# taindp98/Endoscopy-Image-Classification

Measured on AMD Instinct MI355X. Metric: unlabeled images/sec/node (FixMatch ViT-S, 224², μ=7), higher is better.
Workload: dtype bf16; 1 GPU; F1: FixMatch ViT-S/16 step, global B=64 labeled + mu*B=448 unlabeled weak/strong pairs (64 + 448 per GPU, strong scaling), 224^2, C=23, tau=0.95, lambda_u=1, Adam 1e-3, EMA 0.999; global_batch=960, seq_len=197, parallelism=dp1, hipgraph=False

## Files before the change

endoscopy-image-classification_amd/csrc/gemm.hip:

```cpp
#include <algorithm>
#include <cstdlib>

#include <hip/hip_ext.h>

#include "common.h"

namespace es_gemm {

constexpr int BM = 128, BN = 128, BK = 64;

enum Epi {
  EPI_BF16 = 0,
  EPI_GELU = 1,
  EPI_F32_RESID = 2,
  EPI_DGELU = 3,
  EPI_F32 = 4,
  EPI_PATCH = 5,
  EPI_GELU_ACT = 6,
  EPI_GELU_D = 7,
  EPI_MULAUX = 8,
};

struct NTArgs {
  const bf16* A; const bf16* B; const float* bias;
  void* C; void* C2; const void* aux;
  int M, N, K, lda, ldb, ldc, ldaux, np;
};

__device__ __forceinline__ int swz128(int r, int c) { return c ^ ((r >> 1) & 7); }
__device__ __forceinline__ int swz64(int r, int c) { return c ^ ((4 - ((r >> 2) & 3)) & 3); }

template <int EPI>
struct EpiCtx {
  __amdgpu_buffer_rsrc_t c, c2, aux;
// ... 1293 lines not shown
    if (d == (int)gridDim.x - 1) {
      for (int x = 0; x < 8; ++x)
        for (int c = 0; c < ncg; ++c) __hip_atomic_store(ctr + x * 8 + c, 0, __ATOMIC_RELAXED, __HIP_MEMORY_SCOPE_AGENT);
      __hip_atomic_store(ctr + SLOT_INTS - 1, 0, __ATOMIC_RELAXED, __HIP_MEMORY_SCOPE_AGENT);
    }
  }
}

namespace rlg {
constexpr int R = 32, KD = 384, D = 384;
constexpr int ROWA = KD * 2, TA = R * ROWA;
constexpr int ROWX = D * 4, TX = R * ROWX;
constexpr int STAGE = TA + TX, NST = 2;
constexpr int PA = TA / 1024 / 8, PX = TX / 1024 / 8;
constexpr int QN = 4;
constexpr int LDS = NST * STAGE + QN * 4 + 16 + D * 4 * 3;
constexpr int SLOTS = 64, SLOT_INTS = 4;
}
__device__ int g_rl_ctr[rlg::SLOTS * rlg::SLOT_INTS];

__device__ __forceinline__ float sq2_rounded(float a, float b) {
#pragma clang fp contract(off)
  return a * a + b * b;
}
__device__ __forceinline__ float sq2_fused(float a, float b) {
#pragma clang fp contract(off)
  return __builtin_fmaf(a, a, b * b);
}
__device__ __forceinline__ float mul_rounded(float a, float b) {
#pragma clang fp contract(off)
  return a * b;
}

struct RLArgs {
  const float* gamma; const float* beta;
  bf16* h; float* mean; float* rstd;
  int ldh; float eps;
};

__global__ __launch_bounds__(512, 1) void gemm_resid_ln_kernel(NTArgs p, RLArgs l, int slot) {
  using namespace rlg;
  extern __shared__ __attribute__((aligned(16))) char smem[];
  int* const qring = (int*)(smem + NST * STAGE);
  float* const bias_lds = (float*)(qring + QN + 4);
  float* const gam_lds = bias_lds + D;
  float* const bet_lds = gam_lds + D;
  const int tid = threadIdx.x, lane = tid & 63;
  const int w = __builtin_amdgcn_readfirstlane(tid >> 6);
  const int g = lane >> 4, r = lane & 15;
  int* const ctr = g_rl_ctr + slot * SLOT_INTS;
  const int nt = (p.M + R - 1) / R;
  if (tid == 0) {
    qring[0] = __hip_atomic_fetch_add(ctr, 1, __ATOMIC_RELAXED, __HIP_MEMORY_SCOPE_AGENT);
    qring[1] = __hip_atomic_fetch_add(ctr, 1, __ATOMIC_RELAXED, __HIP_MEMORY_SCOPE_AGENT);
  }
  bf16x8 wf[3][12];
  const int nw = w * 48;
#pragma unroll
  for (int j = 0; j < 3; ++j)
#pragma unroll
    for (int kk = 0; kk < 12; ++kk)
      wf[j][kk] = *(const bf16x8*)(p.B + (size_t)(nw + 16 * j + r) * p.ldb + 32 * kk + 8 * g);
  if (tid < D / 4) {
    *(f32x4*)(bias_lds + 4 * tid) = p.bias ? *(const f32x4*)(p.bias + 4 * tid) : f32x4{0.f, 0.f, 0.f, 0.f};
    *(f32x4*)(gam_lds + 4 * tid) = *(const f32x4*)(l.gamma + 4 * tid);
    *(f32x4*)(bet_lds + 4 * tid) = *(const f32x4*)(l.beta + 4 * tid);
// ... 72 lines not shown
        seq += 1;
        after_claim = seq;
      }
      char* S = smem + st * STAGE;
      unsigned xb4[4];
#pragma unroll
      for (int k = 0; k < 4; ++k)
        xb4[k] = (unsigned)(uintptr_t)(const __attribute__((address_space(3))) void*)(S + xbase[k]);
      f32x4 acc[2][3];
      ws_mfma_half<0>(acc, wf, xb4);
      ws_mfma_half<1>(acc, wf, xb4);
      char* X = S + TA;
#pragma unroll
      for (int a = 0; a < 2; ++a)
#pragma unroll
        for (int j = 0; j < 3; ++j) {
          const int row = 16 * a + r, c = w * 12 + 4 * j + g;
          f32x4* q = (f32x4*)(X + row * ROWX + ((c ^ r) << 4));
          const f32x4 v = acc[a][j] + *(const f32x4*)(bias_lds + nw + 16 * j + 4 * g);
          *q = v + *q;
        }
      asm volatile("s_waitcnt lgkmcnt(0)" ::: "memory");
      __builtin_amdgcn_s_barrier();
      const int m0 = cur * R;
#pragma unroll
      for (int q = 0; q < 4; ++q) {
        const int row = w * 4 + q;
        float2 v[3];
#pragma unroll
        for (int j = 0; j < 3; ++j) {
          const int cc = (j * 64 + lane) >> 1;
          v[j] = *(const float2*)(X + row * ROWX + ((cc ^ (row & 15)) << 4) + (lane & 1) * 8);
        }
        float s = 0.f;
#pragma unroll
        for (int j = 0; j < 3; ++j) s += v[j].x + v[j].y;
        const float mean = warp_sum(s) * (1.0f / D);
        float a[3], b[3];
#pragma unroll
        for (int j = 0; j < 3; ++j) {
          a[j] = v[j].x - mean;
          b[j] = v[j].y - mean;
        }
        const bool even = (q & 1) == 0;
        const float t0 = even ? sq2_fused(a[0], b[0]) : sq2_rounded(a[0], b[0]);
        const float t1 = sq2_rounded(a[1], b[1]);
        const float t2 = even ? sq2_fused(a[2], b[2]) : sq2_rounded(a[2], b[2]);
        const float ss = (t0 + t1) + t2;
        const float rstd = 1.0f / sqrtf(__builtin_fmaf(warp_sum(ss), 1.0f / D, l.eps));
        const int m = m0 + row;
        const bool ok = m < p.M;
#pragma unroll
        for (int j = 0; j < 3; ++j) {
          const int c = (j * 64 + lane) * 2;
          const float2 gm = *(const float2*)(gam_lds + c), bt = *(const float2*)(bet_lds + c);
          typedef __bf16 bf16x2 __attribute__((ext_vector_type(2)));
          bf16x2 o = {(bf16)__builtin_fmaf(mul_rounded(a[j], rstd), gm.x, bt.x),
                      (bf16)__builtin_fmaf(mul_rounded(b[j], rstd), gm.y, bt.y)};
          __builtin_amdgcn_raw_buffer_store_b64(__builtin_bit_cast(u32x2, v[j]), rx,
                                                ok ? (unsigned)(m * p.ldc + c) * 4u : ES_OOB, 0, 0);
          __builtin_amdgcn_raw_buffer_store_b32(__builtin_bit_cast(unsigned, o), rh,
                                                ok ? (unsigned)(m * l.ldh + c) * 2u : ES_OOB, 0, 0);
        }
        const bool one = ok && lane == 0;
        __builtin_amdgcn_raw_buffer_store_b32(__builtin_bit_cast(unsigned, mean), rm, one ? (unsigned)m * 4u : ES_OOB,
                                              0, 0);
        __builtin_amdgcn_raw_buffer_store_b32(__builtin_bit_cast(unsigned, rstd), rs, one ? (unsigned)m * 4u : ES_OOB,
                                              0, 0);
      }
      seq += 4 * 8;
      if (claimer) {
        wait_vmcnt_any(seq - after_claim);
        asm volatile("" : "+v"(claimed));
        const int c2 = __builtin_amdgcn_readfirstlane(claimed);
        if (lane == 0) qring[(it + 2) & (QN - 1)] = c2;
      }
      st ^= 1;
    }
  }
  asm volatile("s_waitcnt vmcnt(0)" ::: "memory");
  if (tid == 0) {
    const int d = __hip_atomic_fetch_add(ctr + SLOT_INTS - 1, 1, __ATOMIC_RELAXED, __HIP_MEMORY_SCOPE_AGENT);
    if (d == (int)gridDim.x - 1) {
      __hip_atomic_store(ctr, 0, __ATOMIC_RELAXED, __HIP_MEMORY_SCOPE_AGENT);
      __hip_atomic_store(ctr + SLOT_INTS - 1, 0, __ATOMIC_RELAXED, __HIP_MEMORY_SCOPE_AGENT);
    }
  }
}

#define NT_LAUNCH(E, BKT_, NST_, TBM_, ...)                                             \
  {                                                                                        \
    const size_t lds = std::max((size_t)NST_ * (TBM_ + BN) * BKT_ * 2, (size_t)4 * EPI_WAVE_BYTES); \
    allow_lds(gemm_nt_kernel<E, BKT_, NST_, TBM_, ##__VA_ARGS__>, lds);                   \
    hipLaunchKernelGGL(HIP_KERNEL_NAME(gemm_nt_kernel<E, BKT_, NST_, TBM_, ##__VA_ARGS__>), dim3(grid), dim3(256), lds, stream, a); \
    return ES_OK;                                                                          \
  }
#define NT_EPIS(BKT_, NST_, TBM_, ...)                                            \
  switch (epi) {                                                                  \
    case EPI_BF16: NT_LAUNCH(EPI_BF16, BKT_, NST_, TBM_, ##__VA_ARGS__)           \
    case EPI_GELU: NT_LAUNCH(EPI_GELU, BKT_, NST_, TBM_, ##__VA_ARGS__)           \
    case EPI_F32_RESID: NT_LAUNCH(EPI_F32_RESID, BKT_, NST_, TBM_, ##__VA_ARGS__) \
    case EPI_DGELU: NT_LAUNCH(EPI_DGELU, BKT_, NST_, TBM_, ##__VA_ARGS__)         \
    case EPI_F32: NT_LAUNCH(EPI_F32, BKT_, NST_, TBM_, ##__VA_ARGS__)             \
    case EPI_PATCH: NT_LAUNCH(EPI_PATCH, BKT_, NST_, TBM_, ##__VA_ARGS__)         \
    case EPI_GELU_ACT: NT_LAUNCH(EPI_GELU_ACT, BKT_, NST_, TBM_, ##__VA_ARGS__)   \
    case EPI_GELU_D: NT_LAUNCH(EPI_GELU_D, BKT_, NST_, TBM_, ##__VA_ARGS__)       \
    case EPI_MULAUX: NT_LAUNCH(EPI_MULAUX, BKT_, NST_, TBM_, ##__VA_ARGS__)       \
    default: return ES_BAD_ARG;                                                   \
  }
int launch_nt(int cfg, int epi, int grid, hipStream_t stream, const NTArgs& a) {
  if (cfg == 11 && epi == EPI_F32_RESID) NT_LAUNCH(EPI_F32_RESID, 64, 2, 64, 0)
// ... 69 lines not shown
    (void)hipGetDevice(&dev);
    if (hipDeviceGetAttribute(&cus, hipDeviceAttributeMultiprocessorCount, dev) != hipSuccess || cus <= 0) cus = 256;
  }
  const int ncg = a.N / wsg::NG;
  const int nrt = (a.M + wsg::R - 1) / wsg::R, nch = (nrt + wsg::CH - 1) / wsg::CH;
  const int per = std::max(1, std::min(cus / ncg, nch));
  const int grid = per * ncg;
  const int slot = ws_slot(stream);
  static const int probe = getenv("ENDOSSL_WS_PROBE") ? atoi(getenv("ENDOSSL_WS_PROBE")) : 0;
  if (probe == 5 && epi == EPI_BF16) WS_LAUNCH(EPI_BF16, 0, 5)
  if (probe == 7 && epi == EPI_BF16) WS_LAUNCH(EPI_BF16, 0, 7)
  switch (epi) {
    case EPI_BF16: WS_LAUNCH(EPI_BF16, 0)
    case EPI_GELU: WS_LAUNCH(EPI_GELU, 0)
    case EPI_GELU_ACT: WS_LAUNCH(EPI_GELU_ACT, 0)
    case EPI_GELU_D: WS_LAUNCH(EPI_GELU_D, 0)
    case EPI_F32: WS_LAUNCH(EPI_F32, 0)
    default: return ES_BAD_ARG;
  }
}
#undef WS_LAUNCH

int launch_resid_ln(hipStream_t stream, const NTArgs& a, const RLArgs& l) {
  static int cus = 0;
  if (!cus) {
    int dev = 0;
    (void)hipGetDevice(&dev);
    if (hipDeviceGetAttribute(&cus, hipDeviceAttributeMultiprocessorCount, dev) != hipSuccess || cus <= 0) cus = 256;
  }
  const int nt = (a.M + rlg::R - 1) / rlg::R;
  const int grid = std::max(1, std::min(cus, nt));
  allow_lds(gemm_resid_ln_kernel, (size_t)rlg::LDS);
  hipLaunchKernelGGL(gemm_resid_ln_kernel, dim3(grid), dim3(512), rlg::LDS, stream, a, l, ws_slot(stream));
  return hipGetLastError() == hipSuccess ? ES_OK : ES_HIP_ERROR;
}

}
using namespace es_gemm;

static int g_gemm_variant = -1;
static int g_tn_variant = -1;
static int g_small_tile = 1;


extern "C" {

int endossl_ws_debug_stamps(unsigned long long* host, int n) {
  if (n > WS_DBG) n = WS_DBG;
  return hipMemcpyFromSymbol(host, HIP_SYMBOL(g_ws_dbg), n * sizeof(unsigned long long)) == hipSuccess ? 0 : -3;
}

int es_gemm_tn_ex(const void* A1, int ld1, const void* A2, int ld2, int M, int N1, int N2, int splits,
                  float* workspace, float* out, int accumulate, float* bias_out, int variant, hipStream_t stream);

int es_gemm_nt(int epi, const void* A, int lda, const void* B, int ldb, const float* bias, void* C,
               int ldc, void* C2, const void* aux, int ldaux, int M, int N, int K, int np,
               hipStream_t stream) {
  if (M <= 0 || N <= 0 || K <= 0 || (N % BN) || (K % BK) || (lda % 8) || (ldb % 8) || (ldc % 4))
    return ES_BAD_SHAPE;
  if (!A || !B || !C) return ES_BAD_ARG;
  if (((epi == EPI_GELU || epi == EPI_GELU_D) && !C2) ||
      ((epi == EPI_F32_RESID || epi == EPI_DGELU || epi == EPI_MULAUX || epi == EPI_PATCH) && !aux))
    return ES_BAD_ARG;
  if (epi == EPI_PATCH && np <= 0) return ES_BAD_ARG;
  NTArgs a{(const bf16*)A, (const bf16*)B, bias, C, C2, aux, M, N, K, lda, ldb, ldc, ldaux, np};
  int variant = g_gemm_variant;
// ... 41 lines not shown
      case EPI_GELU_D: L2(EPI_GELU_D)
      case EPI_MULAUX: L2(EPI_MULAUX)
      default: return ES_BAD_ARG;
    }
#undef L2
    return hipGetLastError() == hipSuccess ? ES_OK : ES_HIP_ERROR;
  }
  if (variant == 6 || variant == 10) {
    const int tbn = variant == 6 ? 256 : 128;
    if (N % tbn) return ES_BAD_SHAPE;
    return launch_big(variant, epi, ((M + 255) / 256) * (N / tbn), stream, a);
  }
  if (variant != 0 && variant != 2 && variant != 5 && variant != 11) return ES_BAD_ARG;
  const int tbm = variant == 11 ? 64 : BM;
  const int grid = ((M + tbm - 1) / tbm) * (N / BN);
  const int rc = launch_nt(variant, epi, grid, stream, a);
  if (rc) return rc;
  return hipGetLastError() == hipSuccess ? ES_OK : ES_HIP_ERROR;
}

int es_gemm_nt_resid_ln(const void* A, int lda, const void* B, int ldb, const float* bias, float* C, int ldc,
                        const float* aux, int ldaux, const float* gamma, const float* beta, void* h, int ldh,
                        float* mean, float* rstd, int M, int N, int K, float eps, hipStream_t stream) {
  if (M <= 0 || N != rlg::D || K != rlg::KD || (lda % 8) || (ldb % 8) || (ldc % 2) || (ldaux % 4) || (ldh % 2) ||
      (size_t)M * (size_t)std::max(ldc, ldaux) * 4 >= (1u << 31))
    return ES_BAD_SHAPE;
  if (!A || !B || !C || !aux || !gamma || !beta || !h || !mean || !rstd) return ES_BAD_ARG;
  if ((((uintptr_t)A | (uintptr_t)aux | (uintptr_t)B | (uintptr_t)gamma | (uintptr_t)beta) & 15) ||
      (bias && ((uintptr_t)bias & 15)) || ((uintptr_t)C & 7) || ((uintptr_t)h & 3))
    return ES_BAD_ARG;
  NTArgs a{(const bf16*)A, (const bf16*)B, bias, C, nullptr, aux, M, N, K, lda, ldb, ldc, ldaux, 0};
  RLArgs l{gamma, beta, (bf16*)h, mean, rstd, ldh, eps};
  return launch_resid_ln(stream, a, l);
}

static bool gemm_variant_ok(int v) {
  return v == -1 || v == 0 || v == 1 || v == 2 || v == 5 || v == 6 || v == 10 || v == 11 || v == 12;
}
int es_set_gemm_variant(int v) {
  if (!gemm_variant_ok(v)) return ES_BAD_ARG;
  const int old = g_gemm_variant;
  g_gemm_variant = v;
  return old;
}

int es_set_gemm_small_tile(int v) {
  const int old = g_small_tile;
  g_small_tile = v;
  return old;
}

int es_set_tn_variant(int v) {
  if (v != -1 && v != 0 && v != 7) return ES_BAD_ARG;
  const int old = g_tn_variant;
  g_tn_variant = v;
  return old;
}

constexpr int TN_MIN_SPLIT_TOKENS = 512;
static bool tn_big_ok(int N1, int N2, int ld1, int ld2) {
  return N1 % TB1 == 0 && N2 % TB2 == 0 && ld1 % 8 == 0 && ld2 % 8 == 0;
}
static int tn_pick(int M, int N1, int N2, int ld1, int ld2, int v) {
  if (!(N1 % BM == 0 && N2 % BN == 0)) return 7;
  if (v == 7) return tn_big_ok(N1, N2, ld1, ld2) ? 7 : 0;
  if (v >= 0) return 0;
// ... 261 lines not shown
```

endoscopy-image-classification_amd/endossl/_lib.py:

```python
import ctypes
import os

import torch

_HERE = os.path.dirname(os.path.abspath(__file__))
LIB_PATH = os.environ.get("ENDOSSL_LIB", os.path.join(_HERE, "lib", "libendossl_hip.so"))

V, I, L, F, Z = ctypes.c_void_p, ctypes.c_int, ctypes.c_long, ctypes.c_float, ctypes.c_size_t
U64 = ctypes.c_ulonglong

SIGNATURES = {
    "es_abi_version": (I, []),
    "es_gemm_nt": (I, [I, V, I, V, I, V, V, I, V, V, I, I, I, I, I, V]),
    "es_gemm_nt_resid_ln": (I, [V, I, V, I, V, V, I, V, I, V, V, V, I, V, V, I, I, I, F, V]),
    "es_set_gemm_variant": (I, [I]),
    "es_set_gemm_small_tile": (I, [I]),
    "es_gemm_tn_workspace": (Z, [I, I, I]),
    "es_gemm_tn": (I, [V, I, V, I, I, I, I, I, V, V, I, V, V]),
    "es_gemm_tn_ex": (I, [V, I, V, I, I, I, I, I, V, V, I, V, I, V]),
    "es_set_tn_variant": (I, [I]),
    "es_set_attn_variant": (I, [I]),
    "es_set_attn_bwd_variant": (I, [I]),
    "es_set_attn_bwd_grid": (I, [I]),
    "es_set_ln_fwd_grid": (I, [I]),
    "es_set_attn_bwd_long": (I, [I]),
    "es_splitk_reduce": (I, [V, V, I, I, I, V]),
    "es_tn_problem_size": (Z, []),
    "es_gemm_tn_grouped_prepare": (I, [V, I]),
    "es_gemm_tn_grouped": (I, [V, I, I, V]),
    "es_set_stem_kernels": (I, [I]),
    "es_gemm_tn_big_grouped_table_bytes": (Z, [I]),
    "es_gemm_tn_big_grouped_workspace": (Z, [V, I, I]),
    "es_gemm_tn_big_grouped_prepare": (I, [V, I, I, V, Z, V, V]),
    "es_gemm_tn_big_grouped": (I, [V, I, V, V]),
    "es_gemm_tn_big_grouped_timed": (I, [V, I, V, V, V, V]),
    "es_event_create": (I, [V]),
    "es_event_elapsed": (I, [V, V, V]),
    "es_event_destroy": (I, [V]),
    "es_colsum": (I, [V, I, I, I, V, I, V, I, V]),
    "es_attn_fwd": (I, [V, I, V, I, V, I, I, I, F, V]),
    "es_attn_bwd": (I, [V, I, V, I, V, V, V, I, V, I, I, I, I, F, V]),
    "es_attn_cls_fwd": (I, [V, I, V, I, V, I, I, I, F, V]),
    "es_attn_cls_bwd": (I, [V, I, V, I, V, V, I, V, I, I, I, I, F, V]),
    "es_reduce_partials": (I, [V, V, I, I, I, V]),
    "es_layernorm_fwd": (I, [V, I, V, V, V, I, V, V, I, I, F, V]),
    "es_layernorm_bwd": (I, [V, I, V, I, V, V, V, V, I, V, I, V, I, V, V, V, I, I, I, I, V]),
    "es_layernorm_bwd_b16": (I, [V, I, V, I, V, V, V, V, I, V, I, V, I, V, V, V, I, I, I, I, V]),
# ... 210 lines not shown
```

endoscopy-image-classification_amd/endossl/block.py:

```python
import contextlib
import ctypes

import torch

from . import _lib
from ._lib import ptr, stream

EPI_BF16, EPI_GELU, EPI_F32_RESID, EPI_DGELU, EPI_F32, EPI_PATCH, EPI_GELU_ACT, EPI_GELU_D, EPI_MULAUX = range(9)
ATTN_SCALE = 64 ** -0.5


def gemm_nt(call, epi, a, w, bias, c, M, N, K, c2=None, aux=None, ldc=None, ldaux=None, npatch=0, s=None):
    call("es_gemm_nt", epi, ptr(a), a.stride(0), ptr(w), w.stride(0), ptr(bias), ptr(c), ldc or c.stride(0), ptr(c2),
         ptr(aux), 0 if aux is None else ldaux or aux.stride(0), M, N, K, npatch, stream() if s is None else s)


def gemm_nt_resid_ln(call, a, w, bias, xmid, xin, gamma, beta, h, mean, rstd, M, N, K, eps, s=None):
    call("es_gemm_nt_resid_ln", ptr(a), a.stride(0), ptr(w), w.stride(0), ptr(bias), ptr(xmid), xmid.stride(0),
         ptr(xin), xin.stride(0), ptr(gamma), ptr(beta), ptr(h), h.stride(0), ptr(mean), ptr(rstd), M, N, K, eps,
         stream() if s is None else s)


def layernorm_fwd(call, x, gamma, beta, y, mean, rstd, M, D, eps, s=None):
    call("es_layernorm_fwd", ptr(x), x.stride(0), ptr(gamma), ptr(beta), ptr(y), y.stride(0), ptr(mean), ptr(rstd), M,
         D, eps, stream() if s is None else s)


def layernorm_bwd(call, dy, x, mean, rstd, gamma, dres, dx, dxb, dgamma, dbeta, ws, blocks, M, D, accumulate,
                  lddx=None, s=None):
    call("es_layernorm_bwd_b16" if dy.dtype == torch.bfloat16 else "es_layernorm_bwd", ptr(dy), dy.stride(0), ptr(x),
         x.stride(0), ptr(mean), ptr(rstd), ptr(gamma), ptr(dres), dres.stride(0), ptr(dx), lddx or dx.stride(0),
         ptr(dxb), 0 if dxb is None else dxb.stride(0), ptr(dgamma), ptr(dbeta), ptr(ws), blocks, M, D, accumulate,
         stream() if s is None else s)


def attn_fwd(call, qkv, o, lse, n, T, H, s=None, cls=False):
    call("es_attn_cls_fwd" if cls else "es_attn_fwd", ptr(qkv), qkv.stride(0), ptr(o), o.stride(0), ptr(lse), n, T, H,
         ATTN_SCALE, stream() if s is None else s)


def attn_bwd(call, qkv, o, lse, delta, do, dqkv, n, T, H, s=None):
    call("es_attn_bwd", ptr(qkv), qkv.stride(0), ptr(o), o.stride(0), ptr(lse), ptr(delta), ptr(do), do.stride(0),
         ptr(dqkv), dqkv.stride(0), n, T, H, ATTN_SCALE, stream() if s is None else s)


def attn_cls_bwd(call, qkv, o, lse, do, dqkv, n, T, H, s=None):
    call("es_attn_cls_bwd", ptr(qkv), qkv.stride(0), ptr(o), o.stride(0), ptr(lse), ptr(do), do.stride(0), ptr(dqkv),
         dqkv.stride(0), n, T, H, ATTN_SCALE, stream() if s is None else s)


def cast_f32_bf16(call, src, dst, numel, s=None):
    call("es_cast_f32_bf16", ptr(src), ptr(dst), numel, stream() if s is None else s)


nop = lambda *args: None


class Rows:

    def __init__(self, n, T, H, i0=0, ldx=None, lddxm=None, **bufs):
        self.n, self.T, self.rows, self.ldx, self.lddxm = n, T, n * T, ldx, lddxm
        if i0:
            r0 = i0 * T
            bufs = {k: t[r0 * H:] if k in ("lse", "delta") else t[r0:] for k, t in bufs.items()}
        self.__dict__.update(bufs)


class Chain:

    def __init__(self, call, p, g, wb, wt, heads, eps, gelu_d=True, dh_bf16=True, bracket=lambda lb, fl, f: f()):
        self.call, self.p, self.g, self.wb, self.wt, self.heads, self.eps = call, p, g, wb, wt, heads, eps
        self.gelu_d = gelu_d
        self.epi_dh = EPI_BF16 if dh_bf16 else EPI_F32
        self.bracket = bracket

    def attn_fwd(self, b, R, cls=None, split_q=False):
        call, p, s, M, D = self.call, self.p, stream(), R.rows, R.h1.shape[1]
        layernorm_fwd(call, R.x, p(b + "norm1.weight"), p(b + "norm1.bias"), R.h1, R.mean1, R.rstd1, M, D, self.eps, s)
        w, bias = self.wb[b + "attn.qkv.weight"], p(b + "attn.qkv.bias")
        if cls is not None and split_q:
            gemm_nt(call, EPI_BF16, R.h1, w[D:], bias[D:], R.qkv[:, D:], M, 2 * D, D, s=s)
            cls.h1[:R.n].copy_(R.h1[:M].view(R.n, R.T, D)[:, 0])
            gemm_nt(call, EPI_BF16, cls.h1, w[:D], bias[:D], R.qkv, R.n, D, D, ldc=R.T * 3 * D, s=s)
        else:
            gemm_nt(call, EPI_BF16, R.h1, w, bias, R.qkv, M, 3 * D, D, s=s)
        Ro = R if cls is None else cls
        attn_fwd(call, R.qkv, Ro.o, Ro.lse, R.n, R.T, self.heads, s, cls is not None)

    def mlp_fwd(self, b, R, train, fused=False, label=None):
        call, p, wb, s, M = self.call, self.p, self.wb, stream(), R.rows
        D, Hd = R.h2.shape[1], R.act.shape[1]
        if fused:
            gemm_nt_resid_ln(call, R.o, wb[b + "attn.proj.weight"], p(b + "attn.proj.bias"), R.xmid, R.x,
                             p(b + "norm2.weight"), p(b + "norm2.bias"), R.h2, R.mean2, R.rstd2, M, D, D, self.eps, s)
        else:
            gemm_nt(call, EPI_F32_RESID, R.o, wb[b + "attn.proj.weight"], p(b + "attn.proj.bias"), R.xmid, M, D, D,
                    aux=R.x, ldaux=R.ldx, s=s)
            layernorm_fwd(call, R.xmid, p(b + "norm2.weight"), p(b + "norm2.bias"), R.h2, R.mean2, R.rstd2, M, D,
                          self.eps, s)
        epi, c, c2 = (EPI_GELU_D if self.gelu_d else EPI_GELU, R.pre, R.act) if train else (EPI_GELU_ACT, R.act, None)
        fc1 = lambda: gemm_nt(call, epi, R.h2, wb[b + "mlp.fc1.weight"], p(b + "mlp.fc1.bias"), c, M, Hd, D,
                              c2=c2, s=s)
        self.bracket(label, 2.0 * M * Hd * D, fc1)
        gemm_nt(call, EPI_F32_RESID, R.act, wb[b + "mlp.fc2.weight"], p(b + "mlp.fc2.bias"), R.out, M, D, Hd,
                aux=R.xmid, s=s)

    def mlp_bwd(self, b, R, ln_bwd, wgrad=None, cap=nop, label=None):
        call, p, g, wt, s, M = self.call, self.p, self.g, self.wt, stream(), R.rows
        D, Hd = R.dxb.shape[1], R.dpre.shape[1]
        cap("b_dxb", R.dxb)
        gemm_nt(call, EPI_MULAUX if self.gelu_d else EPI_DGELU, R.dxb, wt[b + "mlp.fc2.weight"], None, R.dpre, M, Hd, D,
                aux=R.pre, s=s)
        if wgrad is not None:
            wgrad(R.dxb, D, R.act, Hd, M, g(b + "mlp.fc2.weight"), g(b + "mlp.fc2.bias"))
        gemm_nt(call, self.epi_dh, R.dpre, wt[b + "mlp.fc1.weight"], None, R.dh, M, D, Hd, s=s)
        if wgrad is not None:
            wgrad(R.dpre, Hd, R.h2, D, M, g(b + "mlp.fc1.weight"), g(b + "mlp.fc1.bias"), label=label)
        cap("b_dpre", R.dpre)
        cap("b_dh2", R.dh)
        ln_bwd(R.dh, R.xmid, R.mean2, R.rstd2, p(b + "norm2.weight"), R.dres, R.dxm, R.dxmb, g(b + "norm2.weight"),
               g(b + "norm2.bias"), M, lddx=R.lddxm)
        gemm_nt(call, EPI_BF16, R.dxmb, wt[b + "attn.proj.weight"], None, R.do, M, D, D, s=s)
        if wgrad is not None:
            wgrad(R.dxmb, D, R.o, D, M, g(b + "attn.proj.weight"), g(b + "attn.proj.bias"))
        cap("b_dxm", R.dxm, R.dxmb)
        cap("b_do", R.do)

    def attn_bwd(self, b, R, ln_bwd, wgrad=None, before_ln1=nop, cap=nop, cls=None, split_q=False):
        call, p, g, s, M, T = self.call, self.p, self.g, stream(), R.rows, R.T
        D = R.dh1.shape[1]
        if cls is None:
            attn_bwd(call, R.qkv, R.o, R.lse, R.delta, R.do, R.dqkv, R.n, T, self.heads, s)
        else:
            attn_cls_bwd(call, R.qkv, cls.o, cls.lse, cls.do, R.dqkv, R.n, T, self.heads, s)
        gemm_nt(call, self.epi_dh, R.dqkv, self.wt[b + "attn.qkv.weight"], None, R.dh1, M, D, 3 * D, s=s)
        if wgrad is not None:
# ... 54 lines not shown
```

endoscopy-image-classification_amd/endossl/vit.py:

```python
import ctypes
import math
import os

import torch
import torch.nn as nn

from . import _lib, block
from ._lib import call, ptr
from .block import (EPI_BF16, EPI_DGELU, EPI_F32, EPI_F32_RESID, EPI_GELU, EPI_GELU_ACT,
                    EPI_GELU_D, EPI_MULAUX, EPI_PATCH, Rows, _TNProblem)

LN_BWD_BLOCKS = 1024
SIDE_PRIORITY = -1
SIDE_PRIORITY_MIN_M = 65536


IMAGENET_MEAN = (0.485, 0.456, 0.406)
IMAGENET_STD = (0.229, 0.224, 0.225)


def _rup(x, m):
    return (x + m - 1) // m * m


# ... 143 lines not shown
        self.dpatch = z(_rup(n * cfg.np, 256), D, dt=b16)
        self.dyn = z(n, D)
        self.delta = z(n * cfg.heads * cfg.T)
        Mc = _rup(n, 256)
        self.c_dx, self.c_dxb = z(Mc, D), z(Mc, D, dt=b16)
        self.c_dpre, self.c_dxmb, self.c_do = z(Mc, Hd, dt=b16), z(Mc, D, dt=b16), z(Mc, D, dt=b16)
        self.c_dh = z(Mc, D, dt=b16) if Engine.DH_BF16 else z(Mc, D)
        self.dxm_cls = z(Mp, D)


class Engine:

    TN_TARGET_BLOCKS = 768
    TN_SHARE = 0.5
    TN_SHARE_MIN_M = 16384
    TN_MAX_SPLITS = 128
    GROUP_WGRAD = "auto"
    GROUP_WGRAD_MAX_M = 16384
    GROUP_LAYERS = 6
    SHARD_LANES = False
    DEFER_LN_GRADS = True
    LN_MULTI_MAX = 32
    LAYER_WGRAD = True
    LAYER_TN_SHARE = 0.375
    _OV = os.environ.get("ENDOSSL_OVERLAP", "1")
    OVERLAP_FWD = _OV in ("1", "fwd")
    OVERLAP = _OV in ("1", "bwd")
    DH_BF16 = True
    GELU_D = True
    PRUNE_LAST = True
    PRUNE_Q = True
    RESID_LN = os.environ.get("ENDOSSL_RESID_LN", "1") == "1"
    RESID_LN_MIN_M = 40000

    PARITY_NAMES = {n: n + "_f32" for n in (
        "es_gemm_nt", "es_gemm_tn", "es_attn_fwd", "es_attn_bwd", "es_attn_cls_fwd", "es_attn_cls_bwd",
        "es_layernorm_fwd", "es_layernorm_bwd", "es_patch_im2col", "es_patch_im2col_u8", "es_embed_bwd",
        "es_pack_weights")}
    PARITY_NAMES.update({"es_layernorm_bwd_b16": "es_layernorm_bwd_f32", "es_cast_f32_bf16": "es_copy_f32"})

    def __init__(self, cfg, device, precision="bf16"):
        if precision not in ("bf16", "fp32"):
            raise ValueError(f"precision must be 'bf16' (production) or 'fp32' (parity mode), got {precision!r}")
        self.cfg, self.device = cfg, device
        self.precision = precision
        self.op_dtype = torch.bfloat16 if precision == "bf16" else torch.float32
        self.layout, self.offs, self.numel = param_layout(cfg)
        self.shapes = dict(self.layout)
        self._acts = {}
        self._grads = {}
        self._ws = None
        self._ws_ln = None
        self._ws_lnp = None
        self._lnp_next = 0
        self._side = None
        self._ncu = None
        self._lane_state, self._gtab = {}, {}
        self._grad_b = None
        self.overlap = self.OVERLAP
        self.overlap_fwd = self.OVERLAP_FWD
        self._packed_version = -1
        D, Hd = cfg.dim, cfg.hidden
        b16 = self.op_dtype
        mats = [("patch_embed.proj.weight", D, 3 * cfg.patch * cfg.patch, False)]
        for i in range(cfg.depth):
            b = f"blocks.{i}."
# ... 84 lines not shown
        if getattr(self, "_third", None) is None:
            self._third = torch.cuda.Stream(device=self.device)
        return self._third

    def forward(self, flat, images_list, train):
        cfg = self.cfg
        s = _lib.stream()
        n = sum(int(t.shape[0]) for t in images_list)
        A = self.acts(n, train)
        D, T, H = cfg.dim, cfg.T, cfg.heads
        K0 = 3 * cfg.patch * cfg.patch
        row = 0
        for t in images_list:
            if t.shape[1:] != (3, cfg.img_size, cfg.img_size) or t.dtype not in (torch.float32, torch.uint8):
                raise ValueError(f"expected fp32 (normalised) or uint8 (raw) [n,3,{cfg.img_size},{cfg.img_size}] "
                                 f"images, got {tuple(t.shape)} {t.dtype}")
            t = t.contiguous()
            if t.dtype == torch.uint8:
                self._call("es_patch_im2col_u8", ptr(t), *IMAGENET_MEAN, *IMAGENET_STD, ptr(A.patches[row * cfg.np:]),
                     int(t.shape[0]), cfg.img_size, cfg.patch, s)
            else:
                self._call("es_patch_im2col", ptr(t), ptr(A.patches[row * cfg.np:]), int(t.shape[0]), cfg.img_size,
                     cfg.patch, s)
            row += int(t.shape[0])
        x0 = A.x[0]
        pos = self.view(flat, "pos_embed")
        block.gemm_nt(self._call, EPI_PATCH, A.patches, self.wb["patch_embed.proj.weight"],
                      self.view(flat, "patch_embed.proj.bias"), x0, n * cfg.np, D, K0, aux=pos, ldaux=D, npatch=cfg.np)
        self._call("es_cls_init", ptr(x0), D, ptr(self.view(flat, "cls_token")), ptr(pos), n, T, D, s)
        M = A.M
        prune = self._prune()
        ch = self._chain(flat)
        fused = self.RESID_LN and D == 384 and self.precision == "bf16" and M >= self.RESID_LN_MIN_M
        for i in range(cfg.depth):
            b = f"blocks.{i}."
            li = i if train else 0
            xin = A.x[i] if train else A.x[i & 1]
            xout = A.x[i + 1] if train else A.x[(i + 1) & 1]
            R = Rows(n, T, H, x=xin, h1=A.h1[li], mean1=A.mean1[li], rstd1=A.rstd1[li], qkv=A.qkv[li], o=A.o[li],
                     lse=A.lse[li], xmid=A.xmid[li], h2=A.h2[li], mean2=A.mean2[li], rstd2=A.rstd2[li],
                     pre=A.pre[li] if train else None, act=A.act[li], out=xout)
            if prune and i == cfg.depth - 1:
                Rc = self._cls_rows(A, n, xin)
                ch.attn_fwd(b, R, cls=Rc, split_q=self.PRUNE_Q)
                ch.mlp_fwd(b, Rc, train)
                if self.capture is not None:
                    self.capture("fwd_cls", train, i, xin[:M], A.c_xout[:n])
                break
            ch.attn_fwd(b, R)
            ch.mlp_fwd(b, R, train, fused=fused, label="fc1_fwd" if train else "fc1_fwd_weak")
            if self.capture is not None:
                self.capture("fwd", train, i, xin[:M], xout[:M])
        xl = A.x[cfg.depth] if train else A.x[cfg.depth & 1]
        Tl = T
        if prune:
            xl, Tl = A.c_xout, 1
        if cfg.head == "emb":
            self._call("es_cls_ln_fwd", ptr(xl), D, Tl, ptr(self.view(flat, "norm.weight")),
                 ptr(self.view(flat, "norm.bias")), ptr(A.fts), D, ptr(A.xhat), ptr(A.rstd_cls), n, D, cfg.eps, s)
            return A.fts
        self._call("es_cls_head_fwd", ptr(xl), D, Tl, ptr(self.view(flat, "norm.weight")), ptr(self.view(flat, "norm.bias")),
             ptr(self.view(flat, "head.weight")), ptr(self.view(flat, "head.bias")), ptr(A.logits),
             cfg.num_classes, ptr(A.xhat), ptr(A.rstd_cls), n, D, cfg.num_classes, cfg.eps, s)
        return A.logits

    def _prune(self):
        return self.PRUNE_LAST

    def _cls_rows(self, A, n, xin=None, G=None):
        T, D = self.cfg.T, self.cfg.dim
        R = Rows(n, 1, self.cfg.heads, ldx=T * D, lddxm=T * D, x=xin, h1=A.c_h1, o=A.c_o, lse=A.c_lse, xmid=A.c_xmid,
                 h2=A.c_h2, mean2=A.c_mean2, rstd2=A.c_rstd2, pre=A.c_pre, act=A.c_act, out=A.c_xout)
        if G is not None:
            R.dxb, R.dpre, R.dh, R.dres, R.dxmb, R.do = G.c_dxb, G.c_dpre, G.c_dh, G.c_dx, G.c_dxmb, G.c_do
            R.dxm = G.dxm_cls
        return R

    def _tn_splits(self, M, N1, N2):
        if self._tn_shared(M, N1, N2):
            if self._ncu is None:
                self._ncu = torch.cuda.get_device_properties(self.device).multi_processor_count
            tiles = (N1 // 384) * (N2 // 192)
            return max(1, int(self._ncu * self.TN_SHARE) // tiles)
# ... 400 lines not shown
```

include/endossl.h:

```cpp
#ifndef ENDOSSL_H
#define ENDOSSL_H
#include <stddef.h>
#include <stdint.h>
#include <hip/hip_runtime_api.h>

#ifdef __cplusplus
extern "C" {
#endif

int es_abi_version(void);

int es_gemm_nt(int epi, const void* A, int lda, const void* B, int ldb, const float* bias, void* C, int ldc,
               void* C2, const void* aux, int ldaux, int M, int N, int K, int np, hipStream_t stream);
int es_gemm_nt_resid_ln(const void* A, int lda, const void* B, int ldb, const float* bias, float* C, int ldc,
                        const float* aux, int ldaux, const float* gamma, const float* beta, void* h, int ldh,
                        float* mean, float* rstd, int M, int N, int K, float eps, hipStream_t stream);
int es_set_gemm_variant(int variant);
int es_set_gemm_small_tile(int v);
int es_set_tn_variant(int variant);
size_t es_gemm_tn_workspace(int N1, int N2, int splits);
int es_gemm_tn(const void* A1, int ld1, const void* A2, int ld2, int M, int N1, int N2, int splits,
               float* workspace, float* out, int accumulate, float* bias_out, hipStream_t stream);
int es_gemm_tn_ex(const void* A1, int ld1, const void* A2, int ld2, int M, int N1, int N2, int splits,
                  float* workspace, float* out, int accumulate, float* bias_out, int variant, hipStream_t stream);
int es_splitk_reduce(const float* P, float* out, int S, int n, int accumulate, hipStream_t stream);
typedef struct {
  const void* dy;
  const void* x;
  float* out;
  float* bias_out;
  int M, N1, N2, ld1, ld2;
  int mchunk, tile0, pad;
} es_tn_problem;
size_t es_tn_problem_size(void);
int es_gemm_tn_grouped_prepare(void* host_table, int count);
int es_gemm_tn_grouped(const void* device_table, int count, int total_tiles, hipStream_t stream);
size_t es_gemm_tn_big_grouped_table_bytes(int count);
size_t es_gemm_tn_big_grouped_workspace(const void* problems, int count, int target_wgs);
int es_gemm_tn_big_grouped_prepare(const void* problems, int count, int target_wgs, float* workspace,
                                   size_t workspace_floats, void* table, int* dims);
int es_gemm_tn_big_grouped(const void* table, int count, const int* dims, hipStream_t stream);
int es_gemm_tn_big_grouped_timed(const void* table, int count, const int* dims, void* start, void* stop,
                                 hipStream_t stream);
int es_event_create(void** ev);
int es_event_elapsed(void* start, void* stop, float* ms);
int es_event_destroy(void* ev);
int es_colsum(const void* Y, int ld, int M, int N, float* workspace, int blocks, float* out, int accumulate,
              hipStream_t stream);
int es_reduce_partials(const float* P, float* out, int G, int N, int accumulate, hipStream_t stream);
// ... 319 lines not shown
```

Before: 15000 unlabeled images/s.

## Fuse fc2 GEMM with residual add and next block's LayerNorm1

Adds a persistent GEMM kernel that computes fc2, adds bias and the residual, writes the fp32 block output, and applies the next block's norm1 LayerNorm in the epilogue, emitting bf16 h1 plus mean/rstd. The Python forward then skips the standalone layernorm_fwd in the following attention block when M is large. This removes a separate LN kernel launch and a full re-read of the fp32 residual stream per block. In exchange the fused kernel uses a full-width N=384 tile with one block per CU and a heavier epilogue, which may reduce GEMM efficiency compared with the generic path.

```diff
diff --git a/endoscopy-image-classification_amd/csrc/gemm.hip b/endoscopy-image-classification_amd/csrc/gemm.hip
--- a/endoscopy-image-classification_amd/csrc/gemm.hip
+++ b/endoscopy-image-classification_amd/csrc/gemm.hip
@@ -1,5 +1,6 @@
 #include <algorithm>
 #include <cstdlib>
+#include <type_traits>
 
 #include <hip/hip_ext.h>
 
@@ -1359,6 +1360,41 @@
   return a * b;
 }
 
+struct LnRow384 {
+  float mean, rstd;
+  unsigned h[3];
+};
+__device__ __forceinline__ LnRow384 ln_row384(const float2 (&v)[3], bool even, float eps, const float* gam_lds,
+                                              const float* bet_lds, int lane) {
+  constexpr int D = 384;
+  LnRow384 o;
+  float s = 0.f;
+#pragma unroll
+  for (int j = 0; j < 3; ++j) s += v[j].x + v[j].y;
+  o.mean = warp_sum(s) * (1.0f / D);
+  float a[3], b[3];
+#pragma unroll
+  for (int j = 0; j < 3; ++j) {
+    a[j] = v[j].x - o.mean;
+    b[j] = v[j].y - o.mean;
+  }
+  const float t0 = even ? sq2_fused(a[0], b[0]) : sq2_rounded(a[0], b[0]);
+  const float t1 = sq2_rounded(a[1], b[1]);
+  const float t2 = even ? sq2_fused(a[2], b[2]) : sq2_rounded(a[2], b[2]);
+  const float ss = (t0 + t1) + t2;
+  o.rstd = 1.0f / sqrtf(__builtin_fmaf(warp_sum(ss), 1.0f / D, eps));
+#pragma unroll
+  for (int j = 0; j < 3; ++j) {
+    const int c = (j * 64 + lane) * 2;
+    const float2 gm = *(const float2*)(gam_lds + c), bt = *(const float2*)(bet_lds + c);
+    typedef __bf16 bf16x2 __attribute__((ext_vector_type(2)));
+    const bf16x2 h = {(bf16)__builtin_fmaf(mul_rounded(a[j], o.rstd), gm.x, bt.x),
+                      (bf16)__builtin_fmaf(mul_rounded(b[j], o.rstd), gm.y, bt.y)};
+    o.h[j] = __builtin_bit_cast(unsigned, h);
+  }
+  return o;
+}
+
 struct RLArgs {
   const float* gamma; const float* beta;
   bf16* h; float* mean; float* rstd;
@@ -1497,41 +1533,21 @@
           const int cc = (j * 64 + lane) >> 1;
           v[j] = *(const float2*)(X + row * ROWX + ((cc ^ (row & 15)) << 4) + (lane & 1) * 8);
         }
-        float s = 0.f;
-#pragma unroll
-        for (int j = 0; j < 3; ++j) s += v[j].x + v[j].y;
-        const float mean = warp_sum(s) * (1.0f / D);
-        float a[3], b[3];
-#pragma unroll
-        for (int j = 0; j < 3; ++j) {
-          a[j] = v[j].x - mean;
-          b[j] = v[j].y - mean;
-        }
-        const bool even = (q & 1) == 0;
-        const float t0 = even ? sq2_fused(a[0], b[0]) : sq2_rounded(a[0], b[0]);
-        const float t1 = sq2_rounded(a[1], b[1]);
-        const float t2 = even ? sq2_fused(a[2], b[2]) : sq2_rounded(a[2], b[2]);
-        const float ss = (t0 + t1) + t2;
-        const float rstd = 1.0f / sqrtf(__builtin_fmaf(warp_sum(ss), 1.0f / D, l.eps));
+        const LnRow384 o = ln_row384(v, (q & 1) == 0, l.eps, gam_lds, bet_lds, lane);
         const int m = m0 + row;
         const bool ok = m < p.M;
 #pragma unroll
         for (int j = 0; j < 3; ++j) {
           const int c = (j * 64 + lane) * 2;
-          const float2 gm = *(const float2*)(gam_lds + c), bt = *(const float2*)(bet_lds + c);
-          typedef __bf16 bf16x2 __attribute__((ext_vector_type(2)));
-          bf16x2 o = {(bf16)__builtin_fmaf(mul_rounded(a[j], rstd), gm.x, bt.x),
-                      (bf16)__builtin_fmaf(mul_rounded(b[j], rstd), gm.y, bt.y)};
           __builtin_amdgcn_raw_buffer_store_b64(__builtin_bit_cast(u32x2, v[j]), rx,
                                                 ok ? (unsigned)(m * p.ldc + c) * 4u : ES_OOB, 0, 0);
-          __builtin_amdgcn_raw_buffer_store_b32(__builtin_bit_cast(unsigned, o), rh,
-                                                ok ? (unsigned)(m * l.ldh + c) * 2u : ES_OOB, 0, 0);
+          __builtin_amdgcn_raw_buffer_store_b32(o.h[j], rh, ok ? (unsigned)(m * l.ldh + c) * 2u : ES_OOB, 0, 0);
         }
         const bool one = ok && lane == 0;
-        __builtin_amdgcn_raw_buffer_store_b32(__builtin_bit_cast(unsigned, mean), rm, one ? (unsigned)m * 4u : ES_OOB,
-                                              0, 0);
-        __builtin_amdgcn_raw_buffer_store_b32(__builtin_bit_cast(unsigned, rstd), rs, one ? (unsigned)m * 4u : ES_OOB,
-                                              0, 0);
+        __builtin_amdgcn_raw_buffer_store_b32(__builtin_bit_cast(unsigned, o.mean), rm,
+                                              one ? (unsigned)m * 4u : ES_OOB, 0, 0);
+        __builtin_amdgcn_raw_buffer_store_b32(__builtin_bit_cast(unsigned, o.rstd), rs,
+                                              one ? (unsigned)m * 4u : ES_OOB, 0, 0);
       }
       seq += 4 * 8;
       if (claimer) {
@@ -1542,6 +1558,202 @@
       }
       st ^= 1;
     }
+  }
+  asm volatile("s_waitcnt vmcnt(0)" ::: "memory");
+  if (tid == 0) {
+    const int d = __hip_atomic_fetch_add(ctr + SLOT_INTS - 1, 1, __ATOMIC_RELAXED, __HIP_MEMORY_SCOPE_AGENT);
+    if (d == (int)gridDim.x - 1) {
+      __hip_atomic_store(ctr, 0, __ATOMIC_RELAXED, __HIP_MEMORY_SCOPE_AGENT);
+      __hip_atomic_store(ctr + SLOT_INTS - 1, 0, __ATOMIC_RELAXED, __HIP_MEMORY_SCOPE_AGENT);
+    }
+  }
+}
+
+namespace nlg {
+constexpr int TBM = 128, D = 384, WN = 4, MF = 4, NF = 6;
+constexpr int SLABR = 64, ROWX = D * 4, SLAB = SLABR * ROWX;
+constexpr int RPS = SLABR / 8;
+constexpr int SLOTS = 64, SLOT_INTS = 4;
+template <int NST, int BKT>
+constexpr int body() { return NST * (TBM + D) * BKT * 2 > SLAB ? NST * (TBM + D) * BKT * 2 : SLAB; }
+template <int NST, int BKT>
+constexpr int lds() { return body<NST, BKT>() + 16 + D * 4 * 3; }
+}
+__device__ int g_nl_ctr[nlg::SLOTS * nlg::SLOT_INTS];
+
+template <int NST, int BKT>
+__global__ __launch_bounds__(512, 1) void gemm_nt_ln_kernel(NTArgs p, RLArgs l, int slot) {
+  using namespace nlg;
+  extern __shared__ __attribute__((aligned(16))) char smem[];
+  constexpr int ROWB = BKT * 2, RPI = 1024 / ROWB, CPR = ROWB / 16, RPW = 8 * RPI;
+  constexpr int IA = TBM / RPW, IB = D / RPW, PER = IA + IB;
+  static_assert(TBM % RPW == 0 && D % RPW == 0, "tile");
+  constexpr int TA = TBM * ROWB, STAGE = (TBM + D) * ROWB;
+  int* const qslot = (int*)(smem + body<NST, BKT>());
+  float* const bias_lds = (float*)(smem + body<NST, BKT>() + 16);
+  float* const gam_lds = bias_lds + D;
+  float* const bet_lds = gam_lds + D;
+  const int tid = threadIdx.x, lane = tid & 63;
+  const int w = __builtin_amdgcn_readfirstlane(tid >> 6);
+  const int wm = w / WN, wn = w % WN;
+  const int g = lane >> 4, r = lane & 15;
+  int* const ctr = g_nl_ctr + slot * SLOT_INTS;
+  const int nt = (p.M + TBM - 1) / TBM;
+  if (tid == 0) qslot[0] = __hip_atomic_fetch_add(ctr, 1, __ATOMIC_RELAXED, __HIP_MEMORY_SCOPE_AGENT);
+  if (tid < D / 4) {
+    *(f32x4*)(bias_lds + 4 * tid) = p.bias ? *(const f32x4*)(p.bias + 4 * tid) : f32x4{0.f, 0.f, 0.f, 0.f};
+    *(f32x4*)(gam_lds + 4 * tid) = *(const f32x4*)(l.gamma + 4 * tid);
+    *(f32x4*)(bet_lds + 4 * tid) = *(const f32x4*)(l.beta + 4 * tid);
+  }
+  __syncthreads();
+  int cur = __builtin_amdgcn_readfirstlane(qslot[0]);
+
+  const bf16* gb[IB];
+  int arow[IA], acol[IA];
+#pragma unroll
+  for (int j = 0; j < IB; ++j) {
+    const int row = (j * 8 + w) * RPI + lane / CPR;
+    gb[j] = p.B + (size_t)row * p.ldb + swzk<BKT>(row, lane % CPR) * 8;
+  }
+#pragma unroll
+  for (int j = 0; j < IA; ++j) {
+    arow[j] = (j * 8 + w) * RPI + lane / CPR;
+    acol[j] = swzk<BKT>(arow[j], lane % CPR) * 8;
+  }
+  const unsigned rows = (unsigned)p.M;
+  const __amdgpu_buffer_rsrc_t rx = buf_rsrc(p.C, rows * p.ldc * 4u);
+  const __amdgpu_buffer_rsrc_t rh = buf_rsrc(l.h, rows * l.ldh * 2u);
+  const __amdgpu_buffer_rsrc_t rm = buf_rsrc(l.mean, rows * 4u);
+  const __amdgpu_buffer_rsrc_t rs = buf_rsrc(l.rstd, rows * 4u);
+  const float* const resid = (const float*)p.aux;
+  const int nk = p.K / BKT;
+
+  while (cur < nt) {
+    const int m0 = cur * TBM, last = p.M - 1;
+    auto tile_row = [&](int s, int q) {
+      const int lr = w * RPS + q;
+      return (lr >> 5) * 64 + s * 32 + (lr & 31);
+    };
+    float2 rv[4][RPS / 2][3];
+    auto load_resid = [&](auto gc) {
+      constexpr int gi = decltype(gc)::value;
+#pragma unroll
+      for (int q = 0; q < RPS / 2; ++q) {
+        const float* xr = resid + (size_t)min(m0 + tile_row(gi >> 1, (gi & 1) * (RPS / 2) + q), last) * p.ldaux;
+#pragma unroll
+        for (int j = 0; j < 3; ++j) rv[gi][q][j] = *(const float2*)(xr + (j * 64 + lane) * 2);
+      }
+    };
+    load_resid(std::integral_constant<int, 0>{});
+
+    const bf16* ga[IA];
+#pragma unroll
+    for (int j = 0; j < IA; ++j) ga[j] = p.A + (size_t)min(m0 + arow[j], last) * p.lda + acol[j];
+#define NL_ISSUE(BUF, K0)                                                                                \
+  {                                                                                                      \
+    char* S_ = smem + (BUF) * STAGE;                                                                     \
+    _Pragma("unroll") for (int j = 0; j < IA; ++j) glds16(ga[j] + (K0), S_ + (j * 8 + w) * 1024);        \
+    _Pragma("unroll") for (int j = 0; j < IB; ++j) glds16(gb[j] + (K0), S_ + TA + (j * 8 + w) * 1024);   \
+  }
+    f32x4 acc[MF][NF];
+#pragma unroll
+    for (int i = 0; i < MF; ++i)
+#pragma unroll
+      for (int j = 0; j < NF; ++j) acc[i][j] = f32x4{0.f, 0.f, 0.f, 0.f};
+#pragma unroll
+    for (int st = 0; st < NST - 1; ++st)
+      if (st < nk) NL_ISSUE(st, st * BKT)
+    int buf = 0;
+    for (int kt = 0; kt < nk; ++kt) {
+      wait_vmcnt(min(NST - 2, nk - 1 - kt) * PER);
+      __builtin_amdgcn_s_barrier();
+      if (kt + NST - 1 < nk) {
+        int nb = buf + NST - 1;
+        nb = nb >= NST ? nb - NST : nb;
+        NL_ISSUE(nb, (kt + NST - 1) * BKT)
+      }
+      const char* As = smem + buf * STAGE;
+      const char* Bs = As + TA;
+#pragma unroll
+      for (int kk = 0; kk < BKT / 32; ++kk) {
+        bf16x8 af[MF], bfr[NF];
+#pragma unroll
+        for (int j = 0; j < NF; ++j) {
+          const int rb = wn * NF * 16 + j * 16 + r;
+          bfr[j] = *(const bf16x8*)(Bs + rb * ROWB + swzk<BKT>(rb, kk * 4 + g) * 16);
+        }
+#pragma unroll
+        for (int i = 0; i < MF; ++i) {
+          const int ra = wm * MF * 16 + i * 16 + r;
+          af[i] = *(const bf16x8*)(As + ra * ROWB + swzk<BKT>(ra, kk * 4 + g) * 16);
+        }
+        __builtin_amdgcn_s_setprio(1);
+#pragma unroll
+        for (int i = 0; i < MF; ++i)
+#pragma unroll
+          for (int j = 0; j < NF; ++j) acc[i][j] = mfma16(bfr[j], af[i], acc[i][j]);
+        __builtin_amdgcn_s_setprio(0);
+      }
+      buf = buf + 1 == NST ? 0 : buf + 1;
+    }
+#undef NL_ISSUE
+    asm volatile("s_waitcnt lgkmcnt(0)" ::: "memory");
+    __builtin_amdgcn_s_barrier();
+    int claimed = 0;
+    if (tid == 0) claimed = __hip_atomic_fetch_add(ctr, 1, __ATOMIC_RELAXED, __HIP_MEMORY_SCOPE_AGENT);
+    load_resid(std::integral_constant<int, 1>{});
+
+    auto slab = [&](auto sc) {
+      constexpr int s = decltype(sc)::value;
+#pragma unroll
+      for (int i = 0; i < 2; ++i)
+#pragma unroll
+        for (int j = 0; j < NF; ++j) {
+          const int lr = wm * 32 + i * 16 + r, c = wn * NF * 4 + 4 * j + g;
+          *(f32x4*)(smem + lr * ROWX + ((c ^ r) << 4)) =
+              acc[2 * s + i][j] + *(const f32x4*)(bias_lds + wn * NF * 16 + 16 * j + 4 * g);
+        }
+      if constexpr (s == 0) load_resid(std::integral_constant<int, 2>{});
+      asm volatile("s_waitcnt lgkmcnt(0)" ::: "memory");
+      __builtin_amdgcn_s_barrier();
+#pragma unroll
+      for (int q = 0; q < RPS; ++q) {
+        const int lr = w * RPS + q;
+        float2 v[3];
+#pragma unroll
+        for (int j = 0; j < 3; ++j) {
+          const int cc = (j * 64 + lane) >> 1;
+          const float2 t = *(const float2*)(smem + lr * ROWX + ((cc ^ (lr & 15)) << 4) + (lane & 1) * 8);
+          const float2 rr = rv[2 * s + q / (RPS / 2)][q % (RPS / 2)][j];
+          v[j] = make_float2(t.x + rr.x, t.y + rr.y);
+        }
+        if constexpr (s == 0)
+          if (q == RPS / 2 - 1) load_resid(std::integral_constant<int, 3>{});
+        const LnRow384 o = ln_row384(v, (q & 1) == 0, l.eps, gam_lds, bet_lds, lane);
+        const int m = m0 + tile_row(s, q);
+        const bool ok = m < p.M;
+#pragma unroll
+        for (int j = 0; j < 3; ++j) {
+          const int c = (j * 64 + lane) * 2;
+          __builtin_amdgcn_raw_buffer_store_b64(__builtin_bit_cast(u32x2, v[j]), rx,
+                                                ok ? (unsigned)(m * p.ldc + c) * 4u : ES_OOB, 0, 0);
+          __builtin_amdgcn_raw_buffer_store_b32(o.h[j], rh, ok ? (unsigned)(m * l.ldh + c) * 2u : ES_OOB, 0, 0);
+        }
+        const bool one = ok && lane == 0;
+        __builtin_amdgcn_raw_buffer_store_b32(__builtin_bit_cast(unsigned, o.mean), rm,
+                                              one ? (unsigned)m * 4u : ES_OOB, 0, 0);
+        __builtin_amdgcn_raw_buffer_store_b32(__builtin_bit_cast(unsigned, o.rstd), rs,
+                                              one ? (unsigned)m * 4u : ES_OOB, 0, 0);
+      }
+    };
+    slab(std::integral_constant<int, 0>{});
+    asm volatile("s_waitcnt lgkmcnt(0)" ::: "memory");
+    __builtin_amdgcn_s_barrier();
+    slab(std::integral_constant<int, 1>{});
+    if (tid == 0) qslot[0] = claimed;
+    asm volatile("s_waitcnt lgkmcnt(0)" ::: "memory");
+    __builtin_amdgcn_s_barrier();
+    cur = __builtin_amdgcn_readfirstlane(qslot[0]);
   }
   asm volatile("s_waitcnt vmcnt(0)" ::: "memory");
   if (tid == 0) {
@@ -1677,6 +1889,27 @@
   const int grid = std::max(1, std::min(cus, nt));
   allow_lds(gemm_resid_ln_kernel, (size_t)rlg::LDS);
   hipLaunchKernelGGL(gemm_resid_ln_kernel, dim3(grid), dim3(512), rlg::LDS, stream, a, l, ws_slot(stream));
+  return hipGetLastError() == hipSuccess ? ES_OK : ES_HIP_ERROR;
+}
+
+int launch_nt_ln(int ring, hipStream_t stream, const NTArgs& a, const RLArgs& l) {
+  static int cus = 0;
+  if (!cus) {
+    int dev = 0;
+    (void)hipGetDevice(&dev);
+    if (hipDeviceGetAttribute(&cus, hipDeviceAttributeMultiprocessorCount, dev) != hipSuccess || cus <= 0) cus = 256;
+  }
+  const int nt = (a.M + nlg::TBM - 1) / nlg::TBM;
+  const int grid = std::max(1, std::min(cus, nt));
+  const int slot = ws_slot(stream);
+  constexpr size_t lds3 = nlg::lds<3, 32>(), lds2 = nlg::lds<2, 64>();
+  if (ring == 1) {
+    allow_lds(gemm_nt_ln_kernel<3, 32>, lds3);
+    hipLaunchKernelGGL(HIP_KERNEL_NAME(gemm_nt_ln_kernel<3, 32>), dim3(grid), dim3(512), lds3, stream, a, l, slot);
+  } else {
+    allow_lds(gemm_nt_ln_kernel<2, 64>, lds2);
+    hipLaunchKernelGGL(HIP_KERNEL_NAME(gemm_nt_ln_kernel<2, 64>), dim3(grid), dim3(512), lds2, stream, a, l, slot);
+  }
   return hipGetLastError() == hipSuccess ? ES_OK : ES_HIP_ERROR;
 }
 
@@ -1784,6 +2017,28 @@
   NTArgs a{(const bf16*)A, (const bf16*)B, bias, C, nullptr, aux, M, N, K, lda, ldb, ldc, ldaux, 0};
   RLArgs l{gamma, beta, (bf16*)h, mean, rstd, ldh, eps};
   return launch_resid_ln(stream, a, l);
+}
+
+static int g_nt_ln_ring = 0;
+int es_gemm_nt_ln(const void* A, int lda, const void* B, int ldb, const float* bias, float* C, int ldc,
+                  const float* aux, int ldaux, const float* gamma, const float* beta, void* h, int ldh, float* mean,
+                  float* rstd, int M, int N, int K, float eps, hipStream_t stream) {
+  if (M <= 0 || N != nlg::D || K <= 0 || (K % 64) || (lda % 8) || (ldb % 8) || (ldc % 2) || (ldaux % 2) || (ldh % 2) ||
+      lda < K || ldb < K || ldc < N || ldaux < N || ldh < N ||
+      (size_t)M * (size_t)std::max(std::max(ldc, ldaux), ldh) * 4 >= (1u << 31))
+    return ES_BAD_SHAPE;
+  if (!A || !B || !C || !aux || !gamma || !beta || !h || !mean || !rstd) return ES_BAD_ARG;
+  if ((((uintptr_t)A | (uintptr_t)B | (uintptr_t)gamma | (uintptr_t)beta) & 15) || (bias && ((uintptr_t)bias & 15)) ||
+      (((uintptr_t)C | (uintptr_t)aux) & 7) || (((uintptr_t)h | (uintptr_t)mean | (uintptr_t)rstd) & 3))
+    return ES_BAD_ARG;
+  NTArgs a{(const bf16*)A, (const bf16*)B, bias, C, nullptr, aux, M, N, K, lda, ldb, ldc, ldaux, 0};
+  RLArgs l{gamma, beta, (bf16*)h, mean, rstd, ldh, eps};
+  return launch_nt_ln(g_nt_ln_ring, stream, a, l);
+}
+int endossl_nt_ln_ring(int v) {
+  const int old = g_nt_ln_ring;
+  g_nt_ln_ring = v == 1 ? 1 : 0;
+  return old;
 }
 
 static bool gemm_variant_ok(int v) {
diff --git a/endoscopy-image-classification_amd/endossl/_lib.py b/endoscopy-image-classification_amd/endossl/_lib.py
--- a/endoscopy-image-classification_amd/endossl/_lib.py
+++ b/endoscopy-image-classification_amd/endossl/_lib.py
@@ -13,6 +13,7 @@
     "es_abi_version": (I, []),
     "es_gemm_nt": (I, [I, V, I, V, I, V, V, I, V, V, I, I, I, I, I, V]),
     "es_gemm_nt_resid_ln": (I, [V, I, V, I, V, V, I, V, I, V, V, V, I, V, V, I, I, I, F, V]),
+    "es_gemm_nt_ln": (I, [V, I, V, I, V, V, I, V, I, V, V, V, I, V, V, I, I, I, F, V]),
     "es_set_gemm_variant": (I, [I]),
     "es_set_gemm_small_tile": (I, [I]),
     "es_gemm_tn_workspace": (Z, [I, I, I]),
diff --git a/endoscopy-image-classification_amd/endossl/block.py b/endoscopy-image-classification_amd/endossl/block.py
--- a/endoscopy-image-classification_amd/endossl/block.py
+++ b/endoscopy-image-classification_amd/endossl/block.py
@@ -18,6 +18,12 @@
 def gemm_nt_resid_ln(call, a, w, bias, xmid, xin, gamma, beta, h, mean, rstd, M, N, K, eps, s=None):
     call("es_gemm_nt_resid_ln", ptr(a), a.stride(0), ptr(w), w.stride(0), ptr(bias), ptr(xmid), xmid.stride(0),
          ptr(xin), xin.stride(0), ptr(gamma), ptr(beta), ptr(h), h.stride(0), ptr(mean), ptr(rstd), M, N, K, eps,
+         stream() if s is None else s)
+
+
+def gemm_nt_ln(call, a, w, bias, xout, xmid, gamma, beta, h, mean, rstd, M, N, K, eps, s=None):
+    call("es_gemm_nt_ln", ptr(a), a.stride(0), ptr(w), w.stride(0), ptr(bias), ptr(xout), xout.stride(0), ptr(xmid),
+         xmid.stride(0), ptr(gamma), ptr(beta), ptr(h), h.stride(0), ptr(mean), ptr(rstd), M, N, K, eps,
          stream() if s is None else s)
 
 
@@ -74,9 +80,11 @@
         self.epi_dh = EPI_BF16 if dh_bf16 else EPI_F32
         self.bracket = bracket
 
-    def attn_fwd(self, b, R, cls=None, split_q=False):
+    def attn_fwd(self, b, R, cls=None, split_q=False, ln_done=False):
         call, p, s, M, D = self.call, self.p, stream(), R.rows, R.h1.shape[1]
-        layernorm_fwd(call, R.x, p(b + "norm1.weight"), p(b + "norm1.bias"), R.h1, R.mean1, R.rstd1, M, D, self.eps, s)
+        if not ln_done:
+            layernorm_fwd(call, R.x, p(b + "norm1.weight"), p(b + "norm1.bias"), R.h1, R.mean1, R.rstd1, M, D,
+                          self.eps, s)
         w, bias = self.wb[b + "attn.qkv.weight"], p(b + "attn.qkv.bias")
         if cls is not None and split_q:
             gemm_nt(call, EPI_BF16, R.h1, w[D:], bias[D:], R.qkv[:, D:], M, 2 * D, D, s=s)
@@ -87,7 +95,7 @@
         Ro = R if cls is None else cls
         attn_fwd(call, R.qkv, Ro.o, Ro.lse, R.n, R.T, self.heads, s, cls is not None)
 
-    def mlp_fwd(self, b, R, train, fused=False, label=None):
+    def mlp_fwd(self, b, R, train, fused=False, label=None, next_ln=None):
         call, p, wb, s, M = self.call, self.p, self.wb, stream(), R.rows
         D, Hd = R.h2.shape[1], R.act.shape[1]
         if fused:
@@ -102,6 +110,11 @@
         fc1 = lambda: gemm_nt(call, epi, R.h2, wb[b + "mlp.fc1.weight"], p(b + "mlp.fc1.bias"), c, M, Hd, D,
                               c2=c2, s=s)
         self.bracket(label, 2.0 * M * Hd * D, fc1)
+        if next_ln is not None:
+            gamma, beta, h1, mean1, rstd1 = next_ln
+            gemm_nt_ln(call, R.act, wb[b + "mlp.fc2.weight"], p(b + "mlp.fc2.bias"), R.out, R.xmid, gamma, beta, h1,
+                       mean1, rstd1, M, D, Hd, self.eps, s)
+            return
         gemm_nt(call, EPI_F32_RESID, R.act, wb[b + "mlp.fc2.weight"], p(b + "mlp.fc2.bias"), R.out, M, D, Hd,
                 aux=R.xmid, s=s)
 
diff --git a/endoscopy-image-classification_amd/endossl/vit.py b/endoscopy-image-classification_amd/endossl/vit.py
--- a/endoscopy-image-classification_amd/endossl/vit.py
+++ b/endoscopy-image-classification_amd/endossl/vit.py
@@ -199,6 +199,10 @@
     PRUNE_Q = True
     RESID_LN = os.environ.get("ENDOSSL_RESID_LN", "1") == "1"
     RESID_LN_MIN_M = 40000
+    FC2_LN = os.environ.get("ENDOSSL_FC2_LN", "1") == "1"
+    FC2_LN_MIN_M = 50000
+    FC2_LN_TRAIN = True
+    FC2_LN_WEAK = True
 
     PARITY_NAMES = {n: n + "_f32" for n in (
         "es_gemm_nt", "es_gemm_tn", "es_attn_fwd", "es_attn_bwd", "es_attn_cls_fwd", "es_attn_cls_bwd",
@@ -349,6 +353,9 @@
         prune = self._prune()
         ch = self._chain(flat)
         fused = self.RESID_LN and D == 384 and self.precision == "bf16" and M >= self.RESID_LN_MIN_M
+        fc2_ln = (self.FC2_LN and (self.FC2_LN_TRAIN if train else self.FC2_LN_WEAK) and D == 384
+                  and self.precision == "bf16" and M >= self.FC2_LN_MIN_M)
+        ln_done = False
         for i in range(cfg.depth):
             b = f"blocks.{i}."
             li = i if train else 0
@@ -359,13 +366,19 @@
                      pre=A.pre[li] if train else None, act=A.act[li], out=xout)
             if prune and i == cfg.depth - 1:
                 Rc = self._cls_rows(A, n, xin)
-                ch.attn_fwd(b, R, cls=Rc, split_q=self.PRUNE_Q)
+                ch.attn_fwd(b, R, cls=Rc, split_q=self.PRUNE_Q, ln_done=ln_done)
                 ch.mlp_fwd(b, Rc, train)
                 if self.capture is not None:
                     self.capture("fwd_cls", train, i, xin[:M], A.c_xout[:n])
                 break
-            ch.attn_fwd(b, R)
-            ch.mlp_fwd(b, R, train, fused=fused, label="fc1_fwd" if train else "fc1_fwd_weak")
+            ch.attn_fwd(b, R, ln_done=ln_done)
+            next_ln = None
+            if fc2_ln and i + 1 < cfg.depth:
+                nb, ni = f"blocks.{i + 1}.", i + 1 if train else 0
+                next_ln = (self.view(flat, nb + "norm1.weight"), self.view(flat, nb + "norm1.bias"), A.h1[ni],
+                           A.mean1[ni], A.rstd1[ni])
+            ch.mlp_fwd(b, R, train, fused=fused, label="fc1_fwd" if train else "fc1_fwd_weak", next_ln=next_ln)
+            ln_done = next_ln is not None
             if self.capture is not None:
                 self.capture("fwd", train, i, xin[:M], xout[:M])
         xl = A.x[cfg.depth] if train else A.x[cfg.depth & 1]
diff --git a/include/endossl.h b/include/endossl.h
--- a/include/endossl.h
+++ b/include/endossl.h
@@ -15,6 +15,9 @@
 int es_gemm_nt_resid_ln(const void* A, int lda, const void* B, int ldb, const float* bias, float* C, int ldc,
                         const float* aux, int ldaux, const float* gamma, const float* beta, void* h, int ldh,
                         float* mean, float* rstd, int M, int N, int K, float eps, hipStream_t stream);
+int es_gemm_nt_ln(const void* A, int lda, const void* B, int ldb, const float* bias, float* C, int ldc,
+                  const float* aux, int ldaux, const float* gamma, const float* beta, void* h, int ldh, float* mean,
+                  float* rstd, int M, int N, int K, float eps, hipStream_t stream);
 int es_set_gemm_variant(int variant);
 int es_set_gemm_small_tile(int v);
 int es_set_tn_variant(int variant);
```

Measured after the change: 15350 unlabeled images/s (median of 6 runs). 2.3% higher.
